# google/sentencepiece

Hardware: NVIDIA H100
Metric: sentences_per_sec (higher is better)
Workload: dtype u8 text / int32 ids / f32+f64 scores

## Files before the change

sentencepiece_b200/csrc/engine.cu:

```cuda
#include <cuda_runtime.h>

#include <algorithm>
#include <atomic>
#include <cfloat>
#include <chrono>
#include <cmath>
#include <cstdio>
#include <cstdlib>
#include <cstring>
#include <mutex>
#include <random>
#include <thread>
#include <string>
#include <unordered_map>
#include <vector>

#include "../../include/spm_b200.h"
#include "bpe_kernel.cuh"
#include "bpe_lane2_kernel.cuh"
#include "device_model.h"
#include "kernels.cuh"
#include "lane_kernel.cuh"
#include "model_reader.h"
#include "order_kernel.cuh"
// ... 718 lines not shown
  for (int w = 0; w < 16; ++w) {
    const uint64_t start = lo + (total - win) * static_cast<uint64_t>(w) / 15;
    for (uint64_t k = 0; k < win; ++k) spaces += bytes[start + k] == ' ';
    seen += win;
  }
  return spaces * 16 >= seen;
}

int spm_engine::pick_fast_words_device(const uint8_t *d_bytes_base, const uint64_t *d_offs, size_t n, cudaStream_t st, bool *fast) {
  *fast = true;
  if (force_fast_words >= 0) { *fast = force_fast_words != 0; return SPM_OK; }
  if (!(km.flags & kFlagFastWords) || n == 0) return SPM_OK;
  CUDA_TRY(d_sample.ensure(2));
  CUDA_TRY(h_ctrl64.ensure(8));
  CUDA_TRY(cudaMemsetAsync(d_sample.p, 0, 2 * sizeof(unsigned long long), st));
  sample_spaces_kernel<<<16, 256, 0, st>>>(d_bytes_base, d_offs, static_cast<uint32_t>(n), d_sample.p);
  CUDA_TRY(cudaGetLastError());
  CUDA_TRY(cudaMemcpyAsync(h_ctrl64.p + 6, d_sample.p, 2 * sizeof(unsigned long long), cudaMemcpyDeviceToHost, st));
  CUDA_TRY(cudaStreamSynchronize(st));
  const unsigned long long spaces = h_ctrl64.p[6], seen = h_ctrl64.p[7];
  *fast = seen < 64 || spaces * 16 >= seen;
  return SPM_OK;
}

int spm_engine::build_order(const uint64_t *d_offs, size_t n, cudaStream_t st, const uint32_t **order, uint32_t seg) {
  *order = nullptr;
  if (!sort_by_length || n <= 64) return SPM_OK;
  const uint32_t n32 = static_cast<uint32_t>(n);
  if (seg == 0 || seg > n32) seg = n32;
  const uint32_t segs = (n32 + seg - 1) / seg;
  CUDA_TRY(d_order.ensure(n));
  CUDA_TRY(d_order_hist.ensure(static_cast<size_t>(segs) * kOrderBuckets));
  CUDA_TRY(cudaMemsetAsync(d_order_hist.p, 0, static_cast<size_t>(segs) * kOrderBuckets * sizeof(uint32_t), st));
  const uint32_t per_block = kOrderThreads * kOrderPerThread;
  const dim3 grid((seg + per_block - 1) / per_block, segs);
  order_hist_kernel<<<grid, kOrderThreads, 0, st>>>(d_offs, n32, seg, d_order_hist.p);
  order_scan_kernel<<<segs, kOrderBuckets, 0, st>>>(d_order_hist.p);
  order_scatter_kernel<<<grid, kOrderThreads, 0, st>>>(d_offs, n32, seg, d_order_hist.p, d_order.p);
  CUDA_TRY(cudaGetLastError());
  last_launches += 3;
  *order = d_order.p;
  return SPM_OK;
}

int spm_engine::run_device(const uint8_t *d_bytes_base, const uint64_t *d_offs, size_t n, uint64_t total_bytes,
                           bool spans, int32_t *user_ids, uint64_t user_ids_cap, unsigned long long *user_id_offsets,
                           uint64_t *total_ids, uint64_t *total_norm, cudaStream_t st, DevBuf<int32_t> *out_ids,
                           DevBuf<unsigned long long> *out_offs, unsigned long long off_base) {
  last_launches = 0;
  last_deferred = 0;
  const uint32_t n32 = static_cast<uint32_t>(n);
  const bool bpe = model.model_type == SPM_BPE;
  const int tile_threads = std::min(threads, 512);
  const uint32_t K = km.match_slots;
  const LaneGeom lg = spans ? LaneGeom{} : lane_geometry();
  const bool lane_path = lg.ok;
  LaunchGeom geom = plan_geometry(*this, bpe ? bpe_tile_bytes(ncap, spans) : tile_bytes_for(ncap, K, spans), tile_threads / 32);
  if (lane_path) {
    geom.tiles = lg.threads / 32;
    geom.tile_bytes = lg.warp_bytes;
    geom.hot_link = geom.hot_val = 0;
    geom.smem_bytes = lg.smem;
    const size_t warps_total = static_cast<size_t>(sm_count) * ctas_per_sm * geom.tiles;
    CUDA_TRY(ensure_lane_slabs(warps_total, lane_cap));
    if (bpe) CUDA_TRY(d_bpe_long.ensure(warps_total * bpe_long_bytes(lane_cap)));
  }
  if (geom.smem_bytes > smem_optin) { set_error("shared-memory geometry does not fit; lower smem_norm_cap"); return SPM_ERR_ARG; }
  KModel M = km;
  M.hot_link = geom.hot_link;
  M.hot_val = geom.hot_val;

  unsigned long long tmp_cap = total_bytes + 4ull * n + 1024;
  unsigned long long norm_cap = spans ? (total_bytes * 2 + 8ull * n + 1024) : 0;
  CUDA_TRY(d_sent_start.ensure(n));
  CUDA_TRY(d_sent_count.ensure(n));
  CUDA_TRY(d_deferred.ensure(2 * n + 2));
  CUDA_TRY(d_ctrl32.ensure(16));
  CUDA_TRY(d_deferred2.ensure(2 * n + 2));
  CUDA_TRY(d_ctrl64.ensure(4));
  CUDA_TRY(h_ctrl32.ensure(16));
  CUDA_TRY(h_ctrl64.ensure(4));
  if (spans) {
    CUDA_TRY(d_norm_start.ensure(n));
    CUDA_TRY(d_norm_len.ensure(n));
  }

  const int grid = sm_count * ctas_per_sm;
  for (int attempt = 0; attempt < 3; ++attempt) {
    CUDA_TRY(d_tmp_ids.ensure(tmp_cap));
    if (spans) {
      CUDA_TRY(d_tmp_tok_end.ensure(tmp_cap));
      CUDA_TRY(d_tmp_norm.ensure(norm_cap));
      CUDA_TRY(d_tmp_n2o.ensure(norm_cap));
    }
    CUDA_TRY(cudaMemsetAsync(d_ctrl32.p, 0, 16 * sizeof(uint32_t), st));
    CUDA_TRY(cudaMemsetAsync(d_ctrl64.p, 0, 4 * sizeof(unsigned long long), st));
    KBatch B{};
    B.bytes = d_bytes_base;
    B.offsets = d_offs;
    B.n = n32;
    B.off_lo = cur_off_lo;
    B.off_hi = cur_off_hi;
    B.tmp_ids = d_tmp_ids.p;
    B.tmp_tok_end = d_tmp_tok_end.p;
    B.tmp_cap = tmp_cap;
    B.cursor = d_ctrl64.p;
    B.sent_start = d_sent_start.p;
    B.sent_count = d_sent_count.p;
    B.tmp_norm = d_tmp_norm.p;
    B.tmp_n2o = d_tmp_n2o.p;
    B.tmp_norm_cap = norm_cap;
    B.norm_start = d_norm_start.p;
    B.norm_len = d_norm_len.p;
    B.work_counter = d_ctrl32.p + 4;
    B.deferred = d_deferred.p;
    B.status = d_ctrl32.p;
    B.ncap = ncap;
    B.tile_bytes = geom.tile_bytes;

    CUDA_TRY(cudaEventRecord(ev[0], st));
    if (kstats) {
      CUDA_TRY(d_kstats.ensure(16));
      CUDA_TRY(cudaMemsetAsync(d_kstats.p, 0, 16 * sizeof(unsigned long long), st));
      B.kstats = d_kstats.p;
    }
    if (lane_path) {
      const int rc = build_order(d_offs, n, st, &B.order, cur_ready ? (1u << cur_piece_shift) : 0u);
      if (rc) return rc;
      B.ready = cur_ready;
      B.ready_base = cur_ready_base;
      B.piece_shift = cur_piece_shift;
      launch_lane_encode(lg, grid, M, B, st);
    } else if (bpe) {
      if (spans) encode_bpe_kernel<true><<<grid, tile_threads, geom.smem_bytes, st>>>(M, B);
      else encode_bpe_kernel<false><<<grid, tile_threads, geom.smem_bytes, st>>>(M, B);
    } else if (spans) {
      encode_unigram_kernel<true><<<grid, tile_threads, geom.smem_bytes, st>>>(M, B);
    } else {
      encode_unigram_kernel<false><<<grid, tile_threads, geom.smem_bytes, st>>>(M, B);
    }
    CUDA_TRY(cudaGetLastError());
    ++last_launches;
    CUDA_TRY(cudaEventRecord(ev[1], st));
    CUDA_TRY(cudaMemcpyAsync(h_ctrl32.p, d_ctrl32.p, 16 * sizeof(uint32_t), cudaMemcpyDeviceToHost, st));
    CUDA_TRY(cudaMemcpyAsync(h_ctrl64.p, d_ctrl64.p, 4 * sizeof(unsigned long long), cudaMemcpyDeviceToHost, st));
    CUDA_TRY(cudaStreamSynchronize(st));
    if (kstats) {
      unsigned long long ks[16];
      CUDA_TRY(cudaMemcpy(ks, d_kstats.p, sizeof ks, cudaMemcpyDeviceToHost));
      if (ks[12])
        fprintf(stderr, "[kstats] groups %llu: warp trips/group %.1f, lane trips/sentence %.1f (lane utilisation of K2 %.3f), starts/sentence "
                "%.1f (whole words %.1f), normalized bytes/sentence %.1f (U+2581 as one byte)\n", ks[12], double(ks[8]) / ks[12], double(ks[9]) / n,
                double(ks[9]) / (32.0 * ks[8]), double(ks[10]) / n, double(ks[11]) / n, double(ks[13]) / n);
      if (ks[4]) {
        const double w = 1e-6 / (static_cast<double>(grid) * geom.tiles);
        fprintf(stderr, "[kstats] M cycles per warp (lane 0): group loop %.2f = K1 %.2f, K2 %.2f, K4 %.2f, rest %.2f\n", ks[4] * w,
                ks[5] * w, ks[6] * w, ks[7] * w, (ks[4] - ks[5] - ks[6] - ks[7]) * w);
      }
    }
    uint32_t n_def = h_ctrl32.p[0];
    const uint32_t *def_list = d_deferred.p;
    const LaunchGeom g2 = n_def && lane_path ? plan_geometry(*this, bpe ? bpe_tile_bytes(ncap, false)
                                                                       : tile_bytes_for(ncap, K, false), tile_threads / 32)
                                             : LaunchGeom{};
    if (n_def && lane_path && g2.smem_bytes <= smem_optin) {
      last_deferred = n_def;
      KModel M2 = km;
      M2.hot_link = g2.hot_link;
      M2.hot_val = g2.hot_val;
      KBatch B2 = B;
      B2.sub_list = d_deferred.p;
      B2.sub_n = n_def;
      B2.deferred = d_deferred2.p;
      B2.status = d_ctrl32.p + 8;
      B2.work_counter = d_ctrl32.p + 12;
      B2.ncap = ncap;
      B2.tile_bytes = g2.tile_bytes;
      const int grid2 = static_cast<int>(std::min<uint32_t>(static_cast<uint32_t>(grid), (n_def + g2.tiles - 1) / g2.tiles));
      if (bpe) encode_bpe_kernel<false><<<grid2, tile_threads, g2.smem_bytes, st>>>(M2, B2);
      else encode_unigram_kernel<false><<<grid2, tile_threads, g2.smem_bytes, st>>>(M2, B2);
      CUDA_TRY(cudaGetLastError());
      ++last_launches;
      CUDA_TRY(cudaMemcpyAsync(h_ctrl32.p, d_ctrl32.p, 16 * sizeof(uint32_t), cudaMemcpyDeviceToHost, st));
      CUDA_TRY(cudaMemcpyAsync(h_ctrl64.p, d_ctrl64.p, 4 * sizeof(unsigned long long), cudaMemcpyDeviceToHost, st));
      CUDA_TRY(cudaStreamSynchronize(st));
      n_def = h_ctrl32.p[8];
      h_ctrl32.p[1] |= h_ctrl32.p[9];
      h_ctrl32.p[2] |= h_ctrl32.p[10];
      def_list = d_deferred2.p;
      M.hot_link = M2.hot_link;
      M.hot_val = M2.hot_val;
    }
    if (n_def) {
      last_deferred = std::max<uint64_t>(last_deferred, n_def);
      CUDA_TRY(h_deferred.ensure(2 * static_cast<size_t>(n_def)));
      CUDA_TRY(cudaMemcpyAsync(h_deferred.p, def_list, 2ull * n_def * sizeof(uint32_t), cudaMemcpyDeviceToHost, st));
      std::vector<uint64_t> two(2);
      std::vector<unsigned long long> offs(n_def + 1, 0);
      CUDA_TRY(cudaStreamSynchronize(st));
      for (uint32_t k = 0; k < n_def; ++k) {
        uint32_t need = h_deferred.p[2 * k + 1];
        if (need == 0) {
          const uint32_t s = h_deferred.p[2 * k];
          CUDA_TRY(cudaMemcpy(two.data(), d_offs + s, 16, cudaMemcpyDeviceToHost));
          const uint64_t len = two[1] - two[0];
          const uint64_t bound = (len * max_expand_num + max_expand_den - 1) / max_expand_den + 8;
          if (bound > 0x7FFFFF00ull) { set_error("sentence too long for the device path"); return SPM_ERR_UNSUPPORTED; }
          need = static_cast<uint32_t>(bound);
        }
        need += 8;
        h_deferred.p[2 * k + 1] = need;
        const uint32_t lk = bpe ? 1 : K;
        const unsigned long long bytes = bpe ? bpe_tile_bytes(need, spans) : tile_bytes_for(need, lk, spans);
        offs[k + 1] = offs[k] + ((bytes + 255ull) & ~255ull);
      }
      CUDA_TRY(d_long_scratch.ensure(offs[n_def] + 256));
      CUDA_TRY(d_long_list.ensure(2 * static_cast<size_t>(n_def)));
      CUDA_TRY(d_long_off.ensure(n_def + 1));
      CUDA_TRY(cudaMemcpyAsync(d_long_list.p, h_deferred.p, 2ull * n_def * sizeof(uint32_t), cudaMemcpyHostToDevice, st));
      CUDA_TRY(cudaMemcpyAsync(d_long_off.p, offs.data(), (n_def + 1) * sizeof(unsigned long long), cudaMemcpyHostToDevice, st));
      B.long_list = d_long_list.p;
      B.long_n = n_def;
      B.long_scratch = d_long_scratch.p;
      B.long_scratch_off = d_long_off.p;
      const int lgrid = static_cast<int>(std::min<uint32_t>((n_def + 7) / 8, static_cast<uint32_t>(sm_count) * 4));
      const uint32_t lsmem = 16 + (M.hot_link + M.hot_val) * 4;
      if (bpe) {
        if (spans) encode_bpe_long_kernel<true><<<lgrid, 256, lsmem, st>>>(M, B);
        else encode_bpe_long_kernel<false><<<lgrid, 256, lsmem, st>>>(M, B);
      } else {
        if (spans) encode_unigram_long_kernel<true><<<lgrid, 256, lsmem, st>>>(M, B);
        else encode_unigram_long_kernel<false><<<lgrid, 256, lsmem, st>>>(M, B);
      }
      CUDA_TRY(cudaGetLastError());
      ++last_launches;
      CUDA_TRY(cudaMemcpyAsync(h_ctrl32.p, d_ctrl32.p, 16 * sizeof(uint32_t), cudaMemcpyDeviceToHost, st));
      CUDA_TRY(cudaMemcpyAsync(h_ctrl64.p, d_ctrl64.p, 4 * sizeof(unsigned long long), cudaMemcpyDeviceToHost, st));
      CUDA_TRY(cudaStreamSynchronize(st));
      h_ctrl32.p[1] |= h_ctrl32.p[9];
      h_ctrl32.p[2] |= h_ctrl32.p[10];
    }
    if (h_ctrl32.p[1]) {
      if (h_ctrl32.p[1] & 8u) set_error("encode failed: a long sentence normalized to more bytes than the scratch sized for it");
      else if (h_ctrl32.p[1] & 2u) set_error("encode failed: the host-to-device copy of a streamed batch made no progress for 3 s");
      else set_error("encode failed: internal consistency check (status " + std::to_string(h_ctrl32.p[1]) + ")");
      return SPM_ERR_ENCODE;
    }
    if (h_ctrl32.p[2]) {
      tmp_cap = h_ctrl64.p[0] + 1024;
      norm_cap = spans ? h_ctrl64.p[1] + 1024 : 0;
      continue;
    }
    break;
  }
  if (h_ctrl32.p[2]) { set_error("temporary buffer overflow persisted"); return SPM_ERR_CAPACITY; }
  const uint32_t nb = (n32 + kScanChunk - 1) / kScanChunk;
  CUDA_TRY(d_block_sums.ensure(nb + 1));
  scan_block_sums_kernel<<<nb, 256, 0, st>>>(d_sent_count.p, n32, d_block_sums.p, 0);
  scan_block_prefix_kernel<<<1, 1024, 0, st>>>(d_block_sums.p, nb, d_ctrl64.p + 2);
  CUDA_TRY(cudaMemcpyAsync(h_ctrl64.p, d_ctrl64.p, 4 * sizeof(unsigned long long), cudaMemcpyDeviceToHost, st));
  CUDA_TRY(cudaStreamSynchronize(st));
  const unsigned long long tot = h_ctrl64.p[2];
  *total_ids = tot;
  if (total_norm) *total_norm = spans ? h_ctrl64.p[1] : 0;
  int32_t *ids_out = user_ids;
  unsigned long long *off_out = user_id_offsets;
  if (!user_ids) {
    DevBuf<int32_t> &ib = out_ids ? *out_ids : d_ids;
    DevBuf<unsigned long long> &ob = out_offs ? *out_offs : d_id_offsets;
    CUDA_TRY(ib.ensure(tot + 1));
    CUDA_TRY(ob.ensure(n + 1));
    ids_out = ib.p;
    off_out = ob.p;
    user_ids_cap = ib.cap;
    if (spans) CUDA_TRY(d_tok_end.ensure(tot + 1));
  } else if (tot > user_ids_cap) {
    set_error("ids_capacity too small: need " + std::to_string(tot));
    return SPM_ERR_CAPACITY;
  }
  scan_write_gather_kernel<int32_t><<<nb, 256, 0, st>>>(d_sent_count.p, n32, d_block_sums.p, off_out, d_sent_start.p,
                                                        d_tmp_ids.p, ids_out,
                                                        spans ? d_tmp_tok_end.p : nullptr, spans ? d_tok_end.p : nullptr,
                                                        user_ids_cap, 0, off_base);
  last_launches += 3;
  if (spans) {
    const unsigned long long tn = h_ctrl64.p[1];
    CUDA_TRY(d_norm.ensure(tn + 1));
    CUDA_TRY(d_n2o.ensure(tn + 1));
    CUDA_TRY(d_norm_offsets.ensure(n + 1));
    CUDA_TRY(d_n2o_offsets.ensure(n + 1));
    scan_block_sums_kernel<<<nb, 256, 0, st>>>(d_norm_len.p, n32, d_block_sums.p, 0);
    scan_block_prefix_kernel<<<1, 1024, 0, st>>>(d_block_sums.p, nb, d_ctrl64.p + 3);
    scan_write_gather_kernel<uint8_t><<<nb, 256, 0, st>>>(d_norm_len.p, n32, d_block_sums.p, d_norm_offsets.p,
                                                          d_norm_start.p, d_tmp_norm.p, d_norm.p, nullptr, nullptr,
                                                          d_norm.cap, 0, 0ull);
    scan_block_sums_kernel<<<nb, 256, 0, st>>>(d_norm_len.p, n32, d_block_sums.p, 1);
    scan_block_prefix_kernel<<<1, 1024, 0, st>>>(d_block_sums.p, nb, d_ctrl64.p + 3);
    scan_write_gather_kernel<uint32_t><<<nb, 256, 0, st>>>(d_norm_len.p, n32, d_block_sums.p, d_n2o_offsets.p,
                                                           d_norm_start.p, d_tmp_n2o.p, d_n2o.p, nullptr, nullptr,
                                                           d_n2o.cap, 1, 0ull);
    last_launches += 6;
  }
  CUDA_TRY(cudaGetLastError());
  CUDA_TRY(cudaEventRecord(ev[2], st));
  return SPM_OK;
}
// ... 1551 lines not shown
```

sentencepiece_b200/csrc/lane_kernel.cuh:

```cuda
#ifndef SPM_B200_LANE_KERNEL_CUH_
#define SPM_B200_LANE_KERNEL_CUH_

#include "kernels.cuh"
#include "drain.cuh"

namespace spm_b200 {

constexpr uint32_t kLaneUnk = 0x3FFFFFu;
constexpr uint32_t kWsByte = 0xFFu;

constexpr uint32_t kLaneTextSlack = 12;
__host__ __device__ inline unsigned long long lane_slab_bytes(uint32_t cap) {
  return (static_cast<unsigned long long>(cap / 4 + kLaneTextSlack) + (cap + 4)) * 32ull * 4ull;
}
constexpr uint32_t kLaneTableBytes = 32 + 4096 + 512 + 16 + 16;

__device__ __forceinline__ void fill_lane_tables(const KModel &M, uint32_t *s_tab) {
  const bool has_cm = M.flags & kFlagHasCharsmap;
  for (uint32_t i = threadIdx.x; i < 8 + 1024 + 128 + 4; i += blockDim.x) {
    uint32_t v;
    if (i < 8) v = M.cm_lead[i];
    else if (i < 8 + 1024) v = M.cm_pair[i - 8];
    else if (i < 8 + 1024 + 128) v = static_cast<uint32_t>(M.cm_solo[i - 8 - 1024]);
    else {
// ... 408 lines not shown
  pos = __shfl_sync(0xFFFFFFFFu, pos, 0);
  *room = pos + total <= B.tmp_cap;
  pos += incl - count;
  if (have && !defer) {
    B.sent_start[sent] = pos;
    B.sent_count[sent] = *room ? count : 0u;
  }
  return pos;
}

template <typename F>
__device__ __forceinline__ bool lane_populate_from(const KModel &M, const LaneCtx &c, uint32_t root, const uint16_t *surf,
                                                   uint32_t bp, uint32_t n, F &&piece) {
  bool has_single = false;
  uint32_t l = root;
  uint32_t clen = 0;
  for (uint32_t kpos = surf[bp]; kpos < n; ++kpos) {
    const uint32_t ch = lane_text_byte_plain(c, kpos);
    const uint32_t v = (l >> kLinkBaseShift) ^ ch;
    l = __ldg(&M.trie_node2[v]).x;
    if ((l & kLinkLabelMask) != ch) break;
    if (kpos + 1 == surf[bp + clen + 1]) ++clen;
    const uint32_t kind = (l >> kLinkKindShift) & 3u;
    if (kind == kKindNone || kind == kKindUnused) continue;
    const uint32_t length = (kpos + 1 == surf[bp + clen]) ? clen : clen + 1;
    const float sc = kind == kKindUserDefined
                         ? static_cast<float>(static_cast<double>(__fmul_rn(static_cast<float>(length), M.max_score)) - 0.1)
                         : __uint_as_float(__ldg(M.trie_val + v));
    if (!piece(length, v, sc)) break;
    has_single |= length == 1;
  }
  return has_single;
}

template <bool kWs1 = false>
__device__ __forceinline__ void lane_finish(const KModel &M, const KBatch &B, const LaneCtx &c, uint32_t n, uint32_t nlog,
                                            uint32_t lane, bool have, bool defer, uint32_t sent, bool bf) {
  const uint32_t max_log = __reduce_max_sync(0xFFFFFFFFu, nlog);
  uint32_t count = 0;
  {
    uint32_t pos_b = n, want = n;
    bool prev_unk = false;
    for (uint32_t tb = (max_log + 3u) & ~3u; tb > 0; tb -= 4) {
      uint32_t ev[4];
#pragma unroll
      for (int j = 0; j < 4; ++j) {
        const uint32_t t = tb - 1 - j;
        ev[j] = t < nlog ? slab_ld(c.log + static_cast<size_t>(t) * 32, c.pol) : 0u;
      }
#pragma unroll
      for (int j = 0; j < 4; ++j) {
        const uint32_t t = tb - 1 - j;
        if (t < nlog) {
          const uint32_t e = ev[j];
          if (pos_b == want) {
            const uint32_t plen = (e >> 24) & 63u;
            const bool isunk = (e & 0x3FFFFFu) == kLaneUnk;
            if (bf) count += !isunk ? 1u : (kWs1 && plen == 1u && lane_text_byte(c, want - 1u) == kWsByte) ? 3u : plen;
            else count += !(isunk && prev_unk);
            prev_unk = isunk;
            want -= plen;
          }
          pos_b -= (e >> 31) ? ((e >> 24) & 63u) : ((e >> 22) & 3u) + 1u;
        }
      }
    }
    if (n && want != 0) { atomicOr(B.status + 1, 1u); count = 0; }
  }
  bool room;
  const unsigned long long pos = lane_claim_output(B, lane, count, have, defer, sent, &room);
  if (room) {
    uint32_t pos_b = n, want = n, w = count;
    bool prev_unk = false;
    for (uint32_t tb = (max_log + 3u) & ~3u; tb > 0; tb -= 4) {
      uint32_t ev[4];
#pragma unroll
      for (int j = 0; j < 4; ++j) {
        const uint32_t t = tb - 1 - j;
        ev[j] = t < nlog ? slab_ld(c.log + static_cast<size_t>(t) * 32, c.pol) : 0u;
      }
#pragma unroll
      for (int j = 0; j < 4; ++j) {
      const uint32_t t = tb - 1 - j;
      if (t < nlog && w > 0) {
        const uint32_t e = ev[j];
        if (pos_b == want) {
          const uint32_t plen = (e >> 24) & 63u;
          const uint32_t idx = e & 0x3FFFFFu;
          const bool isunk = idx == kLaneUnk;
          if (isunk) {
            if (bf) {
              for (uint32_t i = 0; i < plen; ++i) {
                const uint32_t ch = lane_text_byte(c, want - 1 - i);
                if (kWs1 && ch == kWsByte) {
                  __stcs(B.tmp_ids + pos + (--w), __ldg(M.byte_to_id + 0x81));
                  __stcs(B.tmp_ids + pos + (--w), __ldg(M.byte_to_id + 0x96));
                  __stcs(B.tmp_ids + pos + (--w), __ldg(M.byte_to_id + 0xE2));
                } else {
                  __stcs(B.tmp_ids + pos + (--w), __ldg(M.byte_to_id + ch));
                }
              }
            } else if (!prev_unk) {
              __stcs(B.tmp_ids + pos + (--w), M.unk_id);
            }
          } else {
            __stcs(B.tmp_ids + pos + (--w), __ldg((kWs1 ? M.trie_id_ws : M.trie_id) + idx));
          }
          prev_unk = isunk;
          want -= plen;
        }
        pos_b -= (e >> 31) ? ((e >> 24) & 63u) : ((e >> 22) & 3u) + 1u;
      }
      }
    }
  }
  slab_discard(c, lane, (__reduce_max_sync(0xFFFFFFFFu, n) >> 2) + 4u, max_log);
}

constexpr uint32_t kRingBp = 32u * 4u, kRingTag = 32u * 8u;
constexpr uint32_t kRingSlot = 32u * (4u + 4u + 2u), kPlainRingSlot = 32u * (4u + 4u);
__host__ __device__ inline uint32_t lane_ring_bytes(uint32_t R) { return R * kRingSlot; }
__host__ __device__ inline uint32_t lane_plain_ring_bytes(uint32_t R) { return R * kPlainRingSlot; }
static_assert(kRingBp == 128, "ring_ld_bp / ring_st_bp spell the back-pointer displacement as +128");
__device__ __forceinline__ float ring_ld_score(uint32_t a) {
  float v;
  asm volatile("ld.shared.f32 %0, [%1];" : "=f"(v) : "r"(a) : "memory");
  return v;
}
__device__ __forceinline__ uint32_t ring_ld_bp(uint32_t a) {
  uint32_t v;
  asm volatile("ld.shared.u32 %0, [%1+128];" : "=r"(v) : "r"(a) : "memory");
  return v;
}
__device__ __forceinline__ uint32_t ring_ld_tag(uint32_t a) {
  uint16_t v;
  asm volatile("ld.shared.u16 %0, [%1];" : "=h"(v) : "r"(a) : "memory");
  return v;
}
__device__ __forceinline__ void ring_st_score(uint32_t a, float v) {
  asm volatile("st.shared.f32 [%0], %1;" :: "r"(a), "f"(v) : "memory");
}
__device__ __forceinline__ void ring_st_bp(uint32_t a, uint32_t v) {
  asm volatile("st.shared.u32 [%0+128], %1;" :: "r"(a), "r"(v) : "memory");
}
__device__ __forceinline__ void ring_st_tag(uint32_t a, uint32_t v) {
  asm volatile("st.shared.u16 [%0], %1;" :: "r"(a), "h"(static_cast<uint16_t>(v)) : "memory");
}

__device__ __forceinline__ bool score_regular(float x) {
  const uint32_t a = __float_as_uint(x) << 1;
  return a == 0u || a - (0x3A800000u << 1) < ((0x48800000u - 0x3A800000u) << 1);
}

constexpr uint32_t kLogWordStep = 1u << 31;
constexpr uint32_t kWsWord = 0x8196E2u;
__device__ __forceinline__ uint32_t one_char_len_ws1(uint32_t lead) { return lead == kWsByte ? 1u : one_char_len(lead); }

__global__ void __launch_bounds__(1024, 1) encode_unigram_lane_kernel(const KModel M, const KBatch B, uint8_t *slabs,
                                                                       uint32_t cap, uint32_t R) {
  extern __shared__ __align__(128) uint8_t smem[];
  uint32_t *s_tab = reinterpret_cast<uint32_t *>(smem);
  fill_lane_tables(M, s_tab);
  __syncthreads();
  const uint32_t lane = threadIdx.x & 31;
  const uint32_t warp_in_cta = threadIdx.x >> 5;
  const uint32_t warp_global = blockIdx.x * (blockDim.x >> 5) + warp_in_cta;
  const LaneCtx c = lane_ctx(s_tab, slabs, cap, warp_global, lane);
  const uint32_t ring_lo = static_cast<uint32_t>(__cvta_generic_to_shared(smem)) + kLaneTableBytes +
                           warp_in_cta * lane_ring_bytes(R) + lane * 4u;
  const uint32_t ring_span = lane_ring_bytes(R);
  const uint32_t ring_hi = ring_lo + ring_span;
  const uint32_t tag_delta = kRingTag - 2u * lane;
  const uint4 *node4 = M.trie_node4;
  const uint32_t root = __ldg(&node4[0]).x;
  const bool bf = M.flags & kFlagByteFallback;
  const bool regular = M.flags & kFlagRegularScores;
  const bool fastwords = M.flags & kFlagFastWords;

  uint32_t first = 0;
  while (lane_claim_group(B, lane, &first)) {
    LanePhaseClock clk(B);
    lane_wait_input(B, first, lane);
    const bool have = first + lane < B.n;
    const uint32_t sent = have && B.order ? B.order[first + lane] : first + lane;
    uint32_t n = 0;
    bool defer = false;
    if (have) {
      defer = !lane_k1<true>(M, B, c, sent, cap, &n, 0xFFF0u);
      if (defer) lane_defer(B, sent);
    }
    __syncwarp();
    clk.mark();
    uint32_t s = 0, ss = ring_lo, k = 0, l = root, lsafe = 0, mblen = 1, nlog = 0, kb = 0;
    bool has_single = false, done = n == 0;
    bool wstart = fastwords;
    float base = 0.f;
    bool base_regular = regular;
    uint32_t w0 = 0, w1 = 0, w2 = 0, w3 = 0;
    unsigned long long cur = 0;
    auto window_low = [&]() -> unsigned long long {
      const uint32_t sh = (s & 3u) * 8u;
      return static_cast<unsigned long long>(__funnelshift_r(w0, w1, sh)) |
             (static_cast<unsigned long long>(__funnelshift_r(w1, w2, sh)) << 32);
    };
    auto window_high = [&]() -> unsigned long long {
      const uint32_t sh = (s & 3u) * 8u;
      return static_cast<unsigned long long>(__funnelshift_r(w2, w3, sh)) |
             (static_cast<unsigned long long>(w3 >> sh) << 32);
    };
    if (!done) {
      for (uint32_t r = 0; r < R; ++r) ring_st_tag(ring_lo + r * kRingSlot + tag_delta, 0xFFFFu);
      ring_st_score(ring_lo, 0.f);
      w0 = slab_ld(c.text_w + 0, c.pol); w1 = slab_ld(c.text_w + 32, c.pol); w2 = slab_ld(c.text_w + 64, c.pol); w3 = slab_ld(c.text_w + 96, c.pol);
      mblen = one_char_len_ws1(w0 & 0xFFu);
      if (mblen > n) mblen = n;
      cur = window_low();
    }
    const bool kst = B.kstats != nullptr && B.seg_done == nullptr;
    uint32_t st_lane = 0;
    while (__any_sync(0xFFFFFFFFu, !done)) {
      if (!done) {
        ++st_lane;
        bool end_walk = true;
        if (k < n) {
          const uint32_t d = k - s;
          uint32_t ch;
          if (d >= 13u) {
            ch = lane_text_byte(c, k);
          } else {
            if (d == 8u) cur = window_high();
            ch = static_cast<uint32_t>(cur) & 0xFFu;
            cur >>= 8;
          }
          kb = ch;
          const uint32_t v = (l >> kLinkBaseShift) ^ ch;
          const uint4 nd = __ldg(&node4[v]);
          if ((nd.x & kLinkLabelMask) == ch) {
            ++k;
            l = nd.x;
            lsafe = nd.w;
            const uint32_t kind = (nd.x >> kLinkKindShift) & 3u;
            if (kind == kKindNormal || kind == kKindUserDefined) {
              const uint32_t plen = k - s;
              uint32_t sl = ss + plen * kRingSlot;
              if (sl >= ring_hi) sl -= ring_span;
              const float curs = ring_ld_score(sl);
              const bool unset = ring_ld_tag(sl + tag_delta) != k;
              float ns;
              bool better;
              if (kind == kKindNormal && base_regular) {
                const float a = __uint_as_float(nd.z);
                ns = __fadd_rn(a, base);
                const float bb = __fsub_rn(ns, a);
                const float err = __fadd_rn(__fsub_rn(a, __fsub_rn(ns, bb)), __fsub_rn(base, bb));
                better = unset || ns > curs || (ns == curs && err > 0.f);
              } else {
                const double sc = kind == kKindNormal
                                      ? static_cast<double>(__uint_as_float(nd.z))
                                      : static_cast<double>(__fmul_rn(static_cast<float>(plen), M.max_score)) - 0.1;
                const double cand = sc + static_cast<double>(base);
                better = unset || cand > static_cast<double>(curs);
                ns = static_cast<float>(cand);
              }
              if (better) {
                ring_st_score(sl, ns);
                ring_st_bp(sl, (plen << 24) | v);
                ring_st_tag(sl + tag_delta, k);
              }
              has_single |= plen == mblen;
            }
            if (k < n) {
              const uint32_t d2 = k - s;
              if (d2 >= 13u) kb = lane_text_byte(c, k);
              else kb = d2 == 8u ? static_cast<uint32_t>(window_high()) & 0xFFu : static_cast<uint32_t>(cur) & 0xFFu;
              end_walk = !((nd.y >> (kb & 31u)) & 1u);
            }
          }
        }
        if (end_walk) {
          const bool fast = wstart && k > s && ((l >> kLinkKindShift) & 3u) == kKindNormal && (k >= n || kb == kWsByte) &&
                            k <= lsafe;
          const uint32_t s_old = s;
          uint32_t steplog;
          if (fast) {
            ss += (k - s) * kRingSlot;
            if (ss >= ring_hi) ss -= ring_span;
            s = k;
            steplog = kLogWordStep;
          } else {
            uint32_t sl = ss + mblen * kRingSlot;
            if (sl >= ring_hi) sl -= ring_span;
            if (!has_single) {
              const float cand = __fadd_rn(M.unk_score, base);
              if (ring_ld_tag(sl + tag_delta) != s + mblen || cand > ring_ld_score(sl)) {
                ring_st_score(sl, cand);
                ring_st_bp(sl, (mblen << 24) | kLaneUnk);
                ring_st_tag(sl + tag_delta, s + mblen);
              }
            }
            ss = sl;
            s += mblen;
            steplog = (mblen - 1u) << 22;
          }
          slab_st(c.log + static_cast<size_t>(nlog) * 32, ring_ld_bp(ss) | steplog, c.pol);
          ++nlog;
          if (s >= n) {
            done = true;
          } else {
            base = ring_ld_score(ss);
            base_regular = regular && score_regular(base);
            const uint32_t jw = (s >> 2) - (s_old >> 2);
            if (jw == 1u) {
              w0 = w1; w1 = w2; w2 = w3;
              w3 = slab_ld(c.text_w + static_cast<size_t>((s >> 2) + 3) * 32, c.pol);
            } else if (jw == 2u) {
              w0 = w2; w1 = w3;
              w2 = slab_ld(c.text_w + static_cast<size_t>((s >> 2) + 2) * 32, c.pol);
              w3 = slab_ld(c.text_w + static_cast<size_t>((s >> 2) + 3) * 32, c.pol);
            } else if (jw != 0u) {
              const uint32_t *tw = c.text_w + static_cast<size_t>(s >> 2) * 32;
              w0 = slab_ld(tw + 0, c.pol); w1 = slab_ld(tw + 32, c.pol); w2 = slab_ld(tw + 64, c.pol); w3 = slab_ld(tw + 96, c.pol);
            }
            cur = window_low();
            const uint32_t b0 = static_cast<uint32_t>(cur) & 0xFFu;
            wstart = fastwords && b0 == kWsByte;
            mblen = one_char_len_ws1(b0);
            if (mblen > n - s) mblen = n - s;
            k = s;
            l = root;
            has_single = false;
          }
        }
      }
    }
    if (kst) {
      typedef unsigned long long ull;
      uint32_t st_fast = 0;
      for (uint32_t t = 0; t < nlog; ++t) st_fast += slab_ld(c.log + static_cast<size_t>(t) * 32, c.pol) >> 31;
      const uint32_t st_trips = __reduce_max_sync(0xFFFFFFFFu, st_lane);
      st_lane = __reduce_add_sync(0xFFFFFFFFu, st_lane);
      const uint32_t st_starts = __reduce_add_sync(0xFFFFFFFFu, nlog);
      st_fast = __reduce_add_sync(0xFFFFFFFFu, st_fast);
      const uint32_t nb = __reduce_add_sync(0xFFFFFFFFu, n);
      if (lane == 0) {
        atomicAdd(B.kstats + 8, ull(st_trips)); atomicAdd(B.kstats + 9, ull(st_lane)); atomicAdd(B.kstats + 10, ull(st_starts));
        atomicAdd(B.kstats + 11, ull(st_fast)); atomicAdd(B.kstats + 12, ull(1)); atomicAdd(B.kstats + 13, ull(nb));
      }
    }
    clk.mark();
    lane_finish<true>(M, B, c, n, nlog, lane, have, defer, sent, bf);
    clk.mark();
    lane_drain(B, sent, have, lane);
    __syncwarp();
    clk.flush(lane);
  }
}

__global__ void __launch_bounds__(1024, 1) encode_unigram_lane_plain_kernel(const KModel M, const KBatch B, uint8_t *slabs,
                                                                       uint32_t cap, uint32_t R) {
  extern __shared__ __align__(128) uint8_t smem[];
  uint32_t *s_tab = reinterpret_cast<uint32_t *>(smem);
  fill_lane_tables(M, s_tab);
  __syncthreads();
  const uint32_t lane = threadIdx.x & 31;
  const uint32_t warp_in_cta = threadIdx.x >> 5;
  const uint32_t warp_global = blockIdx.x * (blockDim.x >> 5) + warp_in_cta;
  const LaneCtx c = lane_ctx(s_tab, slabs, cap, warp_global, lane);
  const uint32_t ring_lo = static_cast<uint32_t>(__cvta_generic_to_shared(smem)) + kLaneTableBytes +
                           warp_in_cta * lane_plain_ring_bytes(R) + lane * 4u;
  const uint32_t ring_span = lane_plain_ring_bytes(R);
  const uint32_t ring_hi = ring_lo + ring_span;
  const uint2 *node2 = M.trie_node2;
  const uint32_t root = __ldg(&node2[0]).x;
  const bool bf = M.flags & kFlagByteFallback;
  const bool regular = M.flags & kFlagRegularScores;

  uint32_t first = 0;
  while (lane_claim_group(B, lane, &first)) {
    LanePhaseClock clk(B);
    lane_wait_input(B, first, lane);
    const bool have = first + lane < B.n;
    const uint32_t sent = have && B.order ? B.order[first + lane] : first + lane;
    uint32_t n = 0;
    bool defer = false;
    if (have) {
      defer = !lane_k1(M, B, c, sent, cap, &n);
      if (defer) lane_defer(B, sent);
    }
    __syncwarp();
    clk.mark();
    uint32_t s = 0, ss = ring_lo , k = 0, l = root, mblen = 1, nlog = 0;
    bool has_single = false, done = n == 0;
    float base = 0.f;
    bool base_regular = regular;
    uint32_t w0 = 0, w1 = 0, w2 = 0, w3 = 0;
    unsigned long long cur = 0;
    auto window_low = [&]() -> unsigned long long {
      const uint32_t sh = (s & 3u) * 8u;
      return static_cast<unsigned long long>(__funnelshift_r(w0, w1, sh)) |
             (static_cast<unsigned long long>(__funnelshift_r(w1, w2, sh)) << 32);
    };
    auto window_high = [&]() -> unsigned long long {
      const uint32_t sh = (s & 3u) * 8u;
      return static_cast<unsigned long long>(__funnelshift_r(w2, w3, sh)) |
             (static_cast<unsigned long long>(w3 >> sh) << 32);
    };
    if (!done) {
      for (uint32_t r = 0; r < R; ++r) ring_st_bp(ring_lo + r * kPlainRingSlot, 0u);
      ring_st_score(ring_lo, 0.f);
      w0 = slab_ld(c.text_w + 0, c.pol); w1 = slab_ld(c.text_w + 32, c.pol); w2 = slab_ld(c.text_w + 64, c.pol); w3 = slab_ld(c.text_w + 96, c.pol);
      mblen = one_char_len(w0 & 0xFFu);
      if (mblen > n) mblen = n;
      cur = window_low();
    }
    while (__any_sync(0xFFFFFFFFu, !done)) {
      if (!done) {
        bool end_walk = true;
        if (k < n) {
          const uint32_t d = k - s;
          uint32_t ch;
          if (d >= 13u) {
            ch = lane_text_byte(c, k);
          } else {
            if (d == 8u) cur = window_high();
            ch = static_cast<uint32_t>(cur) & 0xFFu;
            cur >>= 8;
          }
          const uint32_t v = (l >> kLinkBaseShift) ^ ch;
          const uint2 nd = __ldg(&node2[v]);
          if ((nd.x & kLinkLabelMask) == ch) {
            ++k;
            l = nd.x;
            const uint32_t kind = (nd.x >> kLinkKindShift) & 3u;
            if (kind == kKindNormal || kind == kKindUserDefined) {
              const uint32_t plen = k - s;
              uint32_t sl = ss + plen * kPlainRingSlot;
              if (sl >= ring_hi) sl -= ring_span;
              const float curs = ring_ld_score(sl);
              const bool unset = ring_ld_bp(sl) == 0u;
              float ns;
              bool better;
              if (kind == kKindNormal && base_regular) {
                const float a = __uint_as_float(__ldg(M.trie_val + v));
                ns = __fadd_rn(a, base);
                const float bb = __fsub_rn(ns, a);
                const float err = __fadd_rn(__fsub_rn(a, __fsub_rn(ns, bb)), __fsub_rn(base, bb));
                better = unset || ns > curs || (ns == curs && err > 0.f);
              } else {
                const double sc = kind == kKindNormal
                                      ? static_cast<double>(__uint_as_float(__ldg(M.trie_val + v)))
                                      : static_cast<double>(__fmul_rn(static_cast<float>(plen), M.max_score)) - 0.1;
                const double cand = sc + static_cast<double>(base);
                better = unset || cand > static_cast<double>(curs);
                ns = static_cast<float>(cand);
              }
              if (better) {
                ring_st_score(sl, ns);
                ring_st_bp(sl, (plen << 24) | v);
              }
              has_single |= plen == mblen;
            }
            if (k < n) {
              uint32_t nb;
              const uint32_t d2 = k - s;
              if (d2 >= 13u) nb = lane_text_byte(c, k);
              else nb = d2 == 8u ? static_cast<uint32_t>(window_high()) & 0xFFu : static_cast<uint32_t>(cur) & 0xFFu;
              end_walk = !((nd.y >> (nb & 31u)) & 1u);
            }
          }
        }
        if (end_walk) {
          uint32_t sl = ss + mblen * kPlainRingSlot;
          if (sl >= ring_hi) sl -= ring_span;
          if (!has_single) {
            const float cand = __fadd_rn(M.unk_score, base);
            if (ring_ld_bp(sl) == 0u || cand > ring_ld_score(sl)) {
              ring_st_score(sl, cand);
              ring_st_bp(sl, (mblen << 24) | kLaneUnk);
            }
          }
          ring_st_bp(ss, 0u);
          s += mblen;
          ss = sl;
          slab_st(c.log + static_cast<size_t>(nlog) * 32, ring_ld_bp(ss) | ((mblen - 1u) << 22), c.pol);
          ++nlog;
          if (s >= n) {
            done = true;
          } else {
            base = ring_ld_score(ss);
            base_regular = regular && score_regular(base);
            if ((s >> 2) != ((s - mblen) >> 2)) {
              w0 = w1; w1 = w2; w2 = w3;
              w3 = slab_ld(c.text_w + static_cast<size_t>((s >> 2) + 3) * 32, c.pol);
            }
            cur = window_low();
            mblen = one_char_len(static_cast<uint32_t>(cur) & 0xFFu);
            if (mblen > n - s) mblen = n - s;
            k = s;
            l = root;
            has_single = false;
          }
        }
      }
    }
    clk.mark();
    lane_finish(M, B, c, n, nlog, lane, have, defer, sent, bf);
    clk.mark();
    lane_drain(B, sent, have, lane);
    __syncwarp();
    clk.flush(lane);
  }
}


}
#endif
```

Measured before the change: 221.7 million.

## Batch lane start steps by parking walk-finished lanes until half are ready

Restructures the per-lane unigram Viterbi loop in both lane kernels. Lanes that finish a trie walk now park, and the start-step bookkeeping (ring update, log write, window refill) runs together once at least half of the live lanes are parked. Before, a lane ran the start step as soon as its own walk ended, so the walk and start-step code paths diverged within the warp. This aims to cut that divergence, at the cost of parked lanes idling and an extra ballot per trip. Also adds a kstats counter and print for start steps.

```diff
diff --git a/sentencepiece_b200/csrc/engine.cu b/sentencepiece_b200/csrc/engine.cu
--- a/sentencepiece_b200/csrc/engine.cu
+++ b/sentencepiece_b200/csrc/engine.cu
@@ -894,6 +894,9 @@
         fprintf(stderr, "[kstats] groups %llu: warp trips/group %.1f, lane trips/sentence %.1f (lane utilisation of K2 %.3f), starts/sentence "
                 "%.1f (whole words %.1f), normalized bytes/sentence %.1f (U+2581 as one byte)\n", ks[12], double(ks[8]) / ks[12], double(ks[9]) / n,
                 double(ks[9]) / (32.0 * ks[8]), double(ks[10]) / n, double(ks[11]) / n, double(ks[13]) / n);
+      if (ks[14])
+        fprintf(stderr, "[kstats] start steps/group %.1f, lanes per start step %.1f\n", double(ks[14]) / ks[12],
+                double(ks[10]) / ks[14]);
       if (ks[4]) {
         const double w = 1e-6 / (static_cast<double>(grid) * geom.tiles);
         fprintf(stderr, "[kstats] M cycles per warp (lane 0): group loop %.2f = K1 %.2f, K2 %.2f, K4 %.2f, rest %.2f\n", ks[4] * w,
diff --git a/sentencepiece_b200/csrc/lane_kernel.cuh b/sentencepiece_b200/csrc/lane_kernel.cuh
--- a/sentencepiece_b200/csrc/lane_kernel.cuh
+++ b/sentencepiece_b200/csrc/lane_kernel.cuh
@@ -584,6 +584,10 @@
   return a == 0u || a - (0x3A800000u << 1) < ((0x48800000u - 0x3A800000u) << 1);
 }
 
+constexpr uint32_t kParkNum = 1, kParkDen = 2;
+static_assert(0 < kParkNum && kParkNum <= kParkDen, "the start step must run at the latest when every live lane is parked");
+__device__ __forceinline__ uint32_t park_need(uint32_t live) { return (live * kParkNum + kParkDen - 1u) / kParkDen; }
+
 constexpr uint32_t kLogWordStep = 1u << 31;
 constexpr uint32_t kWsWord = 0x8196E2u;
 __device__ __forceinline__ uint32_t one_char_len_ws1(uint32_t lead) { return lead == kWsByte ? 1u : one_char_len(lead); }
@@ -623,8 +627,8 @@
     }
     __syncwarp();
     clk.mark();
-    uint32_t s = 0, ss = ring_lo, k = 0, l = root, lsafe = 0, mblen = 1, nlog = 0, kb = 0;
-    bool has_single = false, done = n == 0;
+    uint32_t s = 0, ss = ring_lo, k = 0, l = root, lsafe = 0, mblen = 1, nlog = 0, ch = 0;
+    bool has_single = false, parked = false;
     bool wstart = fastwords;
     float base = 0.f;
     bool base_regular = regular;
@@ -640,77 +644,25 @@
       return static_cast<unsigned long long>(__funnelshift_r(w2, w3, sh)) |
              (static_cast<unsigned long long>(w3 >> sh) << 32);
     };
-    if (!done) {
+    if (n != 0) {
       for (uint32_t r = 0; r < R; ++r) ring_st_tag(ring_lo + r * kRingSlot + tag_delta, 0xFFFFu);
       ring_st_score(ring_lo, 0.f);
       w0 = slab_ld(c.text_w + 0, c.pol); w1 = slab_ld(c.text_w + 32, c.pol); w2 = slab_ld(c.text_w + 64, c.pol); w3 = slab_ld(c.text_w + 96, c.pol);
       mblen = one_char_len_ws1(w0 & 0xFFu);
       if (mblen > n) mblen = n;
       cur = window_low();
+      ch = static_cast<uint32_t>(cur) & 0xFFu;
+      cur >>= 8;
     }
     const bool kst = B.kstats != nullptr && B.seg_done == nullptr;
-    uint32_t st_lane = 0;
-    while (__any_sync(0xFFFFFFFFu, !done)) {
-      if (!done) {
-        ++st_lane;
-        bool end_walk = true;
-        if (k < n) {
-          const uint32_t d = k - s;
-          uint32_t ch;
-          if (d >= 13u) {
-            ch = lane_text_byte(c, k);
-          } else {
-            if (d == 8u) cur = window_high();
-            ch = static_cast<uint32_t>(cur) & 0xFFu;
-            cur >>= 8;
-          }
-          kb = ch;
-          const uint32_t v = (l >> kLinkBaseShift) ^ ch;
-          const uint4 nd = __ldg(&node4[v]);
-          if ((nd.x & kLinkLabelMask) == ch) {
-            ++k;
-            l = nd.x;
-            lsafe = nd.w;
-            const uint32_t kind = (nd.x >> kLinkKindShift) & 3u;
-            if (kind == kKindNormal || kind == kKindUserDefined) {
-              const uint32_t plen = k - s;
-              uint32_t sl = ss + plen * kRingSlot;
-              if (sl >= ring_hi) sl -= ring_span;
-              const float curs = ring_ld_score(sl);
-              const bool unset = ring_ld_tag(sl + tag_delta) != k;
-              float ns;
-              bool better;
-              if (kind == kKindNormal && base_regular) {
-                const float a = __uint_as_float(nd.z);
-                ns = __fadd_rn(a, base);
-                const float bb = __fsub_rn(ns, a);
-                const float err = __fadd_rn(__fsub_rn(a, __fsub_rn(ns, bb)), __fsub_rn(base, bb));
-                better = unset || ns > curs || (ns == curs && err > 0.f);
-              } else {
-                const double sc = kind == kKindNormal
-                                      ? static_cast<double>(__uint_as_float(nd.z))
-                                      : static_cast<double>(__fmul_rn(static_cast<float>(plen), M.max_score)) - 0.1;
-                const double cand = sc + static_cast<double>(base);
-                better = unset || cand > static_cast<double>(curs);
-                ns = static_cast<float>(cand);
-              }
-              if (better) {
-                ring_st_score(sl, ns);
-                ring_st_bp(sl, (plen << 24) | v);
-                ring_st_tag(sl + tag_delta, k);
-              }
-              has_single |= plen == mblen;
-            }
-            if (k < n) {
-              const uint32_t d2 = k - s;
-              if (d2 >= 13u) kb = lane_text_byte(c, k);
-              else kb = d2 == 8u ? static_cast<uint32_t>(window_high()) & 0xFFu : static_cast<uint32_t>(cur) & 0xFFu;
-              end_walk = !((nd.y >> (kb & 31u)) & 1u);
-            }
-          }
-        }
-        if (end_walk) {
-          const bool fast = wstart && k > s && ((l >> kLinkKindShift) & 3u) == kKindNormal && (k >= n || kb == kWsByte) &&
+    uint32_t st_lane = 0, st_trips = 0, st_steps = 0;
+    uint32_t need = park_need(__popc(__ballot_sync(0xFFFFFFFFu, s < n)));
+    while (need != 0) {
+      ++st_trips;
+      if (__popc(__ballot_sync(0xFFFFFFFFu, parked)) >= need) {
+        ++st_steps;
+        if (parked) {
+          const bool fast = wstart && k > s && ((l >> kLinkKindShift) & 3u) == kKindNormal && (k >= n || ch == kWsByte) &&
                             k <= lsafe;
           const uint32_t s_old = s;
           uint32_t steplog;
@@ -736,9 +688,7 @@
           }
           slab_st(c.log + static_cast<size_t>(nlog) * 32, ring_ld_bp(ss) | steplog, c.pol);
           ++nlog;
-          if (s >= n) {
-            done = true;
-          } else {
+          if (s < n) {
             base = ring_ld_score(ss);
             base_regular = regular && score_regular(base);
             const uint32_t jw = (s >> 2) - (s_old >> 2);
@@ -754,14 +704,69 @@
               w0 = slab_ld(tw + 0, c.pol); w1 = slab_ld(tw + 32, c.pol); w2 = slab_ld(tw + 64, c.pol); w3 = slab_ld(tw + 96, c.pol);
             }
             cur = window_low();
-            const uint32_t b0 = static_cast<uint32_t>(cur) & 0xFFu;
-            wstart = fastwords && b0 == kWsByte;
-            mblen = one_char_len_ws1(b0);
+            ch = static_cast<uint32_t>(cur) & 0xFFu;
+            cur >>= 8;
+            wstart = fastwords && ch == kWsByte;
+            mblen = one_char_len_ws1(ch);
             if (mblen > n - s) mblen = n - s;
             k = s;
             l = root;
             has_single = false;
           }
+          parked = false;
+        }
+        need = park_need(__popc(__ballot_sync(0xFFFFFFFFu, s < n)));
+      }
+      if (s < n && !parked) {
+        ++st_lane;
+        const uint32_t v = (l >> kLinkBaseShift) ^ ch;
+        const uint4 nd = __ldg(&node4[v]);
+        parked = true;
+        if ((nd.x & kLinkLabelMask) == ch) {
+          ++k;
+          l = nd.x;
+          lsafe = nd.w;
+          const uint32_t kind = (nd.x >> kLinkKindShift) & 3u;
+          if (kind == kKindNormal || kind == kKindUserDefined) {
+            const uint32_t plen = k - s;
+            uint32_t sl = ss + plen * kRingSlot;
+            if (sl >= ring_hi) sl -= ring_span;
+            const float curs = ring_ld_score(sl);
+            const bool unset = ring_ld_tag(sl + tag_delta) != k;
+            float ns;
+            bool better;
+            if (kind == kKindNormal && base_regular) {
+              const float a = __uint_as_float(nd.z);
+              ns = __fadd_rn(a, base);
+              const float bb = __fsub_rn(ns, a);
+              const float err = __fadd_rn(__fsub_rn(a, __fsub_rn(ns, bb)), __fsub_rn(base, bb));
+              better = unset || ns > curs || (ns == curs && err > 0.f);
+            } else {
+              const double sc = kind == kKindNormal
+                                    ? static_cast<double>(__uint_as_float(nd.z))
+                                    : static_cast<double>(__fmul_rn(static_cast<float>(plen), M.max_score)) - 0.1;
+              const double cand = sc + static_cast<double>(base);
+              better = unset || cand > static_cast<double>(curs);
+              ns = static_cast<float>(cand);
+            }
+            if (better) {
+              ring_st_score(sl, ns);
+              ring_st_bp(sl, (plen << 24) | v);
+              ring_st_tag(sl + tag_delta, k);
+            }
+            has_single |= plen == mblen;
+          }
+          if (k < n) {
+            const uint32_t d = k - s;
+            if (d >= 13u) {
+              ch = lane_text_byte(c, k);
+            } else {
+              if (d == 8u) cur = window_high();
+              ch = static_cast<uint32_t>(cur) & 0xFFu;
+              cur >>= 8;
+            }
+            parked = !((nd.y >> (ch & 31u)) & 1u);
+          }
         }
       }
     }
@@ -769,7 +774,6 @@
       typedef unsigned long long ull;
       uint32_t st_fast = 0;
       for (uint32_t t = 0; t < nlog; ++t) st_fast += slab_ld(c.log + static_cast<size_t>(t) * 32, c.pol) >> 31;
-      const uint32_t st_trips = __reduce_max_sync(0xFFFFFFFFu, st_lane);
       st_lane = __reduce_add_sync(0xFFFFFFFFu, st_lane);
       const uint32_t st_starts = __reduce_add_sync(0xFFFFFFFFu, nlog);
       st_fast = __reduce_add_sync(0xFFFFFFFFu, st_fast);
@@ -777,6 +781,7 @@
       if (lane == 0) {
         atomicAdd(B.kstats + 8, ull(st_trips)); atomicAdd(B.kstats + 9, ull(st_lane)); atomicAdd(B.kstats + 10, ull(st_starts));
         atomicAdd(B.kstats + 11, ull(st_fast)); atomicAdd(B.kstats + 12, ull(1)); atomicAdd(B.kstats + 13, ull(nb));
+        atomicAdd(B.kstats + 14, ull(st_steps));
       }
     }
     clk.mark();
@@ -821,8 +826,8 @@
     }
     __syncwarp();
     clk.mark();
-    uint32_t s = 0, ss = ring_lo , k = 0, l = root, mblen = 1, nlog = 0;
-    bool has_single = false, done = n == 0;
+    uint32_t s = 0, ss = ring_lo , k = 0, l = root, mblen = 1, nlog = 0, ch = 0;
+    bool has_single = false, parked = false;
     float base = 0.f;
     bool base_regular = regular;
     uint32_t w0 = 0, w1 = 0, w2 = 0, w3 = 0;
@@ -837,71 +842,20 @@
       return static_cast<unsigned long long>(__funnelshift_r(w2, w3, sh)) |
              (static_cast<unsigned long long>(w3 >> sh) << 32);
     };
-    if (!done) {
+    if (n != 0) {
       for (uint32_t r = 0; r < R; ++r) ring_st_bp(ring_lo + r * kPlainRingSlot, 0u);
       ring_st_score(ring_lo, 0.f);
       w0 = slab_ld(c.text_w + 0, c.pol); w1 = slab_ld(c.text_w + 32, c.pol); w2 = slab_ld(c.text_w + 64, c.pol); w3 = slab_ld(c.text_w + 96, c.pol);
       mblen = one_char_len(w0 & 0xFFu);
       if (mblen > n) mblen = n;
       cur = window_low();
-    }
-    while (__any_sync(0xFFFFFFFFu, !done)) {
-      if (!done) {
-        bool end_walk = true;
-        if (k < n) {
-          const uint32_t d = k - s;
-          uint32_t ch;
-          if (d >= 13u) {
-            ch = lane_text_byte(c, k);
-          } else {
-            if (d == 8u) cur = window_high();
-            ch = static_cast<uint32_t>(cur) & 0xFFu;
-            cur >>= 8;
-          }
-          const uint32_t v = (l >> kLinkBaseShift) ^ ch;
-          const uint2 nd = __ldg(&node2[v]);
-          if ((nd.x & kLinkLabelMask) == ch) {
-            ++k;
-            l = nd.x;
-            const uint32_t kind = (nd.x >> kLinkKindShift) & 3u;
-            if (kind == kKindNormal || kind == kKindUserDefined) {
-              const uint32_t plen = k - s;
-              uint32_t sl = ss + plen * kPlainRingSlot;
-              if (sl >= ring_hi) sl -= ring_span;
-              const float curs = ring_ld_score(sl);
-              const bool unset = ring_ld_bp(sl) == 0u;
-              float ns;
-              bool better;
-              if (kind == kKindNormal && base_regular) {
-                const float a = __uint_as_float(__ldg(M.trie_val + v));
-                ns = __fadd_rn(a, base);
-                const float bb = __fsub_rn(ns, a);
-                const float err = __fadd_rn(__fsub_rn(a, __fsub_rn(ns, bb)), __fsub_rn(base, bb));
-                better = unset || ns > curs || (ns == curs && err > 0.f);
-              } else {
-                const double sc = kind == kKindNormal
-                                      ? static_cast<double>(__uint_as_float(__ldg(M.trie_val + v)))
-                                      : static_cast<double>(__fmul_rn(static_cast<float>(plen), M.max_score)) - 0.1;
-                const double cand = sc + static_cast<double>(base);
-                better = unset || cand > static_cast<double>(curs);
-                ns = static_cast<float>(cand);
-              }
-              if (better) {
-                ring_st_score(sl, ns);
-                ring_st_bp(sl, (plen << 24) | v);
-              }
-              has_single |= plen == mblen;
-            }
-            if (k < n) {
-              uint32_t nb;
-              const uint32_t d2 = k - s;
-              if (d2 >= 13u) nb = lane_text_byte(c, k);
-              else nb = d2 == 8u ? static_cast<uint32_t>(window_high()) & 0xFFu : static_cast<uint32_t>(cur) & 0xFFu;
-              end_walk = !((nd.y >> (nb & 31u)) & 1u);
-            }
-          }
-        }
-        if (end_walk) {
+      ch = static_cast<uint32_t>(cur) & 0xFFu;
+      cur >>= 8;
+    }
+    uint32_t need = park_need(__popc(__ballot_sync(0xFFFFFFFFu, s < n)));
+    while (need != 0) {
+      if (__popc(__ballot_sync(0xFFFFFFFFu, parked)) >= need) {
+        if (parked) {
           uint32_t sl = ss + mblen * kPlainRingSlot;
           if (sl >= ring_hi) sl -= ring_span;
           if (!has_single) {
@@ -916,9 +870,7 @@
           ss = sl;
           slab_st(c.log + static_cast<size_t>(nlog) * 32, ring_ld_bp(ss) | ((mblen - 1u) << 22), c.pol);
           ++nlog;
-          if (s >= n) {
-            done = true;
-          } else {
+          if (s < n) {
             base = ring_ld_score(ss);
             base_regular = regular && score_regular(base);
             if ((s >> 2) != ((s - mblen) >> 2)) {
@@ -926,11 +878,64 @@
               w3 = slab_ld(c.text_w + static_cast<size_t>((s >> 2) + 3) * 32, c.pol);
             }
             cur = window_low();
-            mblen = one_char_len(static_cast<uint32_t>(cur) & 0xFFu);
+            ch = static_cast<uint32_t>(cur) & 0xFFu;
+            cur >>= 8;
+            mblen = one_char_len(ch);
             if (mblen > n - s) mblen = n - s;
             k = s;
             l = root;
             has_single = false;
+          }
+          parked = false;
+        }
+        need = park_need(__popc(__ballot_sync(0xFFFFFFFFu, s < n)));
+      }
+      if (s < n && !parked) {
+        const uint32_t v = (l >> kLinkBaseShift) ^ ch;
+        const uint2 nd = __ldg(&node2[v]);
+        parked = true;
+        if ((nd.x & kLinkLabelMask) == ch) {
+          ++k;
+          l = nd.x;
+          const uint32_t kind = (nd.x >> kLinkKindShift) & 3u;
+          if (kind == kKindNormal || kind == kKindUserDefined) {
+            const uint32_t plen = k - s;
+            uint32_t sl = ss + plen * kPlainRingSlot;
+            if (sl >= ring_hi) sl -= ring_span;
+            const float curs = ring_ld_score(sl);
+            const bool unset = ring_ld_bp(sl) == 0u;
+            float ns;
+            bool better;
+            if (kind == kKindNormal && base_regular) {
+              const float a = __uint_as_float(__ldg(M.trie_val + v));
+              ns = __fadd_rn(a, base);
+              const float bb = __fsub_rn(ns, a);
+              const float err = __fadd_rn(__fsub_rn(a, __fsub_rn(ns, bb)), __fsub_rn(base, bb));
+              better = unset || ns > curs || (ns == curs && err > 0.f);
+            } else {
+              const double sc = kind == kKindNormal
+                                    ? static_cast<double>(__uint_as_float(__ldg(M.trie_val + v)))
+                                    : static_cast<double>(__fmul_rn(static_cast<float>(plen), M.max_score)) - 0.1;
+              const double cand = sc + static_cast<double>(base);
+              better = unset || cand > static_cast<double>(curs);
+              ns = static_cast<float>(cand);
+            }
+            if (better) {
+              ring_st_score(sl, ns);
+              ring_st_bp(sl, (plen << 24) | v);
+            }
+            has_single |= plen == mblen;
+          }
+          if (k < n) {
+            const uint32_t d = k - s;
+            if (d >= 13u) {
+              ch = lane_text_byte(c, k);
+            } else {
+              if (d == 8u) cur = window_high();
+              ch = static_cast<uint32_t>(cur) & 0xFFu;
+              cur >>= 8;
+            }
+            parked = !((nd.y >> (ch & 31u)) & 1u);
           }
         }
       }
```

Result: faster. 242.6 million (median of 6 runs) (+9.4%).
